# Arthur151/ROMP

Measured on NVIDIA H100. Metric: frames/sec 512x512 ROMP-HRNet32 (whole hot path), higher is better.
Workload: dtype bf16

## Files before the change

romp_b200/_lib.py:

```python
from __future__ import annotations

import ctypes as C
import os
import subprocess
import sys

HERE = os.path.dirname(os.path.abspath(__file__))
ROOT = os.path.dirname(HERE)
LIB_PATH = os.path.join(HERE, "lib", "libb200romp.so")
CSRC = os.path.join(HERE, "csrc")
SOURCES = ["net.cu", "conv_simt.cu", "conv_tc.cu", "conv_stem_tc.cu", "conv1d_tc.cu", "parse.cu", "smpl.cu", "smpl_blend_tc.cu", "project.cu", "bev.cu", "pack.cu", "preproc.cu", "temporal.cu", "resnet_ops.cu"]

F32, BF16, U8 = 0, 1, 2
ENGINE_AUTO, ENGINE_SIMT, ENGINE_TCGEN05, ENGINE_TF32 = 0, 1, 2, 3


class ConvDesc(C.Structure):
    _fields_ = [(n, C.c_int) for n in (
        "in_", "in_c_off", "out", "out_c_off", "res", "res_c_off", "res_broadcast", "cin", "cout",
        "ksize", "stride", "relu", "upsample", "input_norm", "pow_channel", "engine")]


class SumDesc(C.Structure):
    _fields_ = [("out", C.c_int), ("base", C.c_int), ("n_terms", C.c_int), ("term", C.c_int * 4), ("up", C.c_int * 4),
                ("relu", C.c_int), ("term_c_off", C.c_int * 4)]


class BevWeights(C.Structure):
    _fields_ = [(n, C.POINTER(C.c_float)) for n in (
        "center_ref", "cam_ref", "coordmap", "anchors", "embed", "w0", "b0", "w1", "b1", "w2", "b2")]


NVCC_FLAGS = ["-Xcompiler", "-fPIC", "-std=c++17", "-O3", "-lineinfo", "-gencode", "arch=compute_90a,code=sm_90a"]
OBJ_DIR = os.path.join(HERE, "lib", "obj")


def _nvcc():
    return os.environ.get("NVCC", "/usr/local/cuda/bin/nvcc")


def nvcc_command(out_path=LIB_PATH):
    return [_nvcc(), "-shared"] + NVCC_FLAGS + ["-o", out_path] + [os.path.join(CSRC, s) for s in SOURCES]


def _headers_mtime():
    hs = [os.path.join(CSRC, f) for f in os.listdir(CSRC) if f.endswith((".cuh", ".h"))]
    hs.append(os.path.join(ROOT, "include", "b200romp.h"))
    return max(os.path.getmtime(h) for h in hs)


def needs_build():
    if not os.path.exists(LIB_PATH):
        return True
    t = os.path.getmtime(LIB_PATH)
    deps = [os.path.join(CSRC, f) for f in os.listdir(CSRC)] + [os.path.join(ROOT, "include", "b200romp.h")]
    return any(os.path.getmtime(d) > t for d in deps)


def build(force=False, verbose=True):
    if not force and not needs_build():
        return LIB_PATH
    from concurrent.futures import ThreadPoolExecutor
    os.makedirs(OBJ_DIR, exist_ok=True)
    hdr_t = _headers_mtime()
    jobs = []
    for s in SOURCES:
        src, obj = os.path.join(CSRC, s), os.path.join(OBJ_DIR, s.replace(".cu", ".o"))
        if force or not os.path.exists(obj) or os.path.getmtime(obj) < max(os.path.getmtime(src), hdr_t):
            jobs.append([_nvcc(), "-c"] + NVCC_FLAGS + ["-o", obj, src])
    if verbose:
        for j in jobs:
            print("[romp_b200] " + " ".join(j), file=sys.stderr)

    def run(cmd):
        r = subprocess.run(cmd, capture_output=True, text=True)
        if r.returncode != 0:
            raise RuntimeError("nvcc failed: " + " ".join(cmd) + "\n" + r.stdout + r.stderr)
        if verbose and r.stderr.strip():
            print(r.stderr, file=sys.stderr)

    with ThreadPoolExecutor(max_workers=min(len(jobs) or 1, os.cpu_count() or 4)) as ex:
        list(ex.map(run, jobs))
    link = [_nvcc(), "-shared", "-gencode", "arch=compute_90a,code=sm_90a", "-o", LIB_PATH] + [os.path.join(OBJ_DIR, s.replace(".cu", ".o")) for s in SOURCES]
    if verbose:
        print("[romp_b200] " + " ".join(link), file=sys.stderr)
    subprocess.run(link, check=True)
    return LIB_PATH


_lib = None


def _sig(fn, restype, *argtypes):
    fn.restype = restype
# ... 84 lines not shown
```

romp_b200/csrc/conv_tc.cuh:

```cuda
#pragma once
#include <cuda.h>

#include <string>
#include <vector>

#include "common.cuh"

namespace b200romp {

struct S2Maps {
  CUtensorMap m[4];
};

struct TcConvPlan {
  int kind = 0;
  int cin = 0, cout = 0, nt = 0;
  int eb = 2;
  int grid_x = 0, grid_y = 0, stages = 0;
  int smem_bytes = 0;
  void* d_wpack = nullptr;
  alignas(64) unsigned char tmap_in[128];
  alignas(64) unsigned char tmap_s2[4][128];
  unsigned kmask = 0xFFFFFFFFu;
  const void* encoded_in = nullptr;
  int encoded_batch = 0;
  std::string describe() const;
};

bool tc_conv_supported(const ConvParams& p, int ksize, int stride);
int tc_conv_prepare(const ConvParams& p, int ksize, int stride, const float* w_oihw, int sm_count, bool ptrs_final, TcConvPlan* plan,
                    std::vector<void*>* allocs);
int tc_conv_launch(const TcConvPlan& plan, const ConvParams& p, cudaStream_t stream);
bool tc_conv1d_supported(const ConvParams& p);
int tc_conv1d_prepare(const ConvParams& p, const float* w_oi3, int sm_count, TcConvPlan* plan, std::vector<void*>* allocs);
int tc_conv1d_launch(TcConvPlan& plan, const ConvParams& p, cudaStream_t stream);
bool tc_stem_supported(const ConvParams& p, int ksize, int stride);
int tc_stem_prepare(const ConvParams& p, const float* w_oihw, int sm_count, bool out_final, TcConvPlan* plan,
                    std::vector<void*>* allocs);
int tc_stem_launch(const TcConvPlan& plan, const ConvParams& p, cudaStream_t stream);

}
```

romp_b200/csrc/net.cu:

```cuda
#include <stdarg.h>
#include <stdlib.h>
#include <string.h>

#include <algorithm>
#include <map>
#include <mutex>
#include <vector>

#include "common.cuh"
#include "conv_tc.cuh"

namespace b200romp {

static thread_local std::string g_last_error;

void set_error(const char* fmt, ...) {
  char buf[1024];
  va_list ap;
  va_start(ap, fmt);
  vsnprintf(buf, sizeof(buf), fmt, ap);
  va_end(ap);
  g_last_error = buf;
}

struct Tensor {
  int H, W, C, dtype, nchw, external;
  void* ptr = nullptr;
  bool constant = false;
  int first_def = -1, last_use = -1;
  size_t frame_bytes() const { return (size_t)H * W * C * dtype_size(dtype); }
};

struct Op {
  int kind = 0;
  b200romp_sum_desc sum;
  b200romp_conv_desc d;
  std::vector<float> w_host, b_host;
  float* d_w_simt = nullptr;
  float* d_bias = nullptr;
  int coutPad = 0;
  int engine = B200ROMP_ENGINE_SIMT;
  TcConvPlan tc;
  int lane = 0;
  int fold = 0;
};

}

using namespace b200romp;

struct b200romp_net {
  int device = 0;
  int sm_count = 132;
  bool finalized = false;
  int max_batch = 0;
  std::vector<Tensor> tensors;
  std::vector<Op> ops;
  std::vector<void*> device_allocs;
  char* workspace = nullptr;
  size_t workspace_bytes = 0;
  struct GraphKey {
    int batch;
    std::vector<void*> ext;
    bool operator<(const GraphKey& o) const { return batch != o.batch ? batch < o.batch : ext < o.ext; }
  };
  std::map<GraphKey, cudaGraphExec_t> graphs;
  bool use_graph = true;
  static constexpr int kLanes = 4;
  cudaStream_t lane_stream[kLanes] = {nullptr, nullptr, nullptr, nullptr};
  std::vector<cudaEvent_t> op_done;
  cudaEvent_t fork_ev = nullptr;
  bool use_lanes = false;
};

static int fill_params(b200romp_net* net, const Op& op, int batch, ConvParams* out) {
  const b200romp_conv_desc& d = op.d;
  const Tensor& ti = net->tensors[d.in];
  const Tensor& to = net->tensors[d.out];
  ConvParams p;
  memset(&p, 0, sizeof(p));
  p.in = ti.ptr; p.out = to.ptr;
  p.w = op.d_w_simt; p.bias = op.d_bias;
  p.B = batch;
  p.Hin = ti.H; p.Win = ti.W; p.in_C = ti.C; p.in_c_off = d.in_c_off; p.cin = d.cin;
  conv_out_hw(d.ksize, d.stride, ti.H, ti.W, &p.Hout, &p.Wout);
  p.out_C = to.C; p.out_c_off = d.out_c_off; p.cout = d.cout; p.coutPad = op.coutPad;
  p.up = d.upsample;
  if (d.res >= 0) {
    const Tensor& tr = net->tensors[d.res];
    p.res = tr.ptr; p.res_C = tr.C; p.res_c_off = op.d.res_c_off; p.res_broadcast = d.res_broadcast;
    p.res_dtype = tr.dtype;
  }
  p.relu = d.relu; p.pow_channel = d.pow_channel; p.out_nchw = to.nchw;
  p.in_dtype = ti.dtype; p.out_dtype = to.dtype; p.input_norm = d.input_norm;
  if (op.fold) {
    p.Win /= 2; p.Wout /= 2;
    p.in_C *= 2; p.cin *= 2; p.out_C *= 2; p.cout *= 2; p.res_C *= 2;
  }
  if (!p.in || !p.out) {
    set_error("op uses an unbound tensor (in=%d out=%d)", d.in, d.out);
    return B200ROMP_ESTATE;
  }
  *out = p;
  return B200ROMP_OK;
}

static int validate_desc(const std::vector<Tensor>& T, const b200romp_conv_desc& d) {
  const int res_c_off = d.res_c_off;
  auto ok_id = [&](int id) { return id >= 0 && id < (int)T.size(); };
  B2R_REQUIRE(ok_id(d.in) && ok_id(d.out) && (d.res == -1 || ok_id(d.res)), "conv: bad tensor id");
  B2R_REQUIRE((d.ksize == 1 || d.ksize == 3 || d.ksize == 7 || (d.ksize == 13 && d.stride == 1 && d.upsample == 1) ||
               (d.ksize == 42 && d.stride == 2 && d.upsample == 1)) && (d.stride == 1 || d.stride == 2),
              "conv: ksize/stride unsupported");
  B2R_REQUIRE(d.upsample == 1 || d.upsample == 2 || d.upsample == 4 || d.upsample == 8, "conv: upsample must be 1,2,4,8");
  const Tensor& ti = T[d.in];
  const Tensor& to = T[d.out];
  B2R_REQUIRE(!ti.nchw, "conv: NCHW inputs unsupported");
  B2R_REQUIRE(d.cin > 0 && d.in_c_off >= 0 && d.in_c_off + d.cin <= ti.C, "conv: input channel slice out of range");
  B2R_REQUIRE(d.cout > 0 && d.out_c_off >= 0 && d.out_c_off + d.cout <= to.C, "conv: output channel slice out of range");
  int Ho, Wo;
  conv_out_hw(d.ksize, d.stride, ti.H, ti.W, &Ho, &Wo);
  B2R_REQUIRE(Ho * d.upsample == to.H && Wo * d.upsample == to.W, "conv: output tensor is %dx%d, op produces %dx%d",
              to.H, to.W, Ho * d.upsample, Wo * d.upsample);
  B2R_REQUIRE(ti.dtype != B200ROMP_U8 || d.input_norm || d.ksize == 7, "conv: u8 input requires input_norm (or the 7x7 stem)");
  B2R_REQUIRE(to.dtype != B200ROMP_U8, "conv: u8 output unsupported");
  B2R_REQUIRE(!to.nchw || to.dtype == B200ROMP_F32, "conv: NCHW output must be fp32");
  if (d.res >= 0) {
// ... 84 lines not shown
  return (int)net->ops.size() - 1;
}

int b200romp_net_add_sum(b200romp_net* net, const b200romp_sum_desc* desc) {
  B2R_REQUIRE(net && desc && !net->finalized, "add_sum: bad arguments or net already finalized");
  const auto& T = net->tensors;
  const int nT = (int)T.size();
  B2R_REQUIRE(desc->out >= 0 && desc->out < nT && desc->base >= 0 && desc->base < nT, "add_sum: tensor id out of range");
  B2R_REQUIRE(desc->n_terms >= 1 && desc->n_terms <= 4, "add_sum: n_terms must be 1..4");
  const Tensor& to = T[desc->out];
  const Tensor& tb = T[desc->base];
  B2R_REQUIRE(!to.nchw && !tb.nchw && to.dtype != B200ROMP_U8 && tb.dtype != B200ROMP_U8, "add_sum: NHWC bf16/fp32 tensors only");
  B2R_REQUIRE(to.C % 8 == 0 && tb.H == to.H && tb.W == to.W && tb.C == to.C, "add_sum: base/out shape mismatch (C %% 8 == 0)");
  for (int k = 0; k < desc->n_terms; ++k) {
    B2R_REQUIRE(desc->term[k] >= 0 && desc->term[k] < nT, "add_sum: term tensor id out of range");
    const Tensor& tt = T[desc->term[k]];
    const int u = desc->up[k];
    B2R_REQUIRE(u == 1 || u == 2 || u == 4 || u == 8, "add_sum: up must be 1,2,4,8");
    const int co = desc->term_c_off[k];
    B2R_REQUIRE(!tt.nchw && tt.dtype != B200ROMP_U8 && tt.C % 8 == 0 && co >= 0 && co % 8 == 0 && co + to.C <= tt.C &&
                    tt.H * u == to.H && tt.W * u == to.W,
                "add_sum: term %d is %dx%dx%d (slice from channel %d), expected %dx%dx%d", k, tt.H, tt.W, tt.C, co, to.H / u, to.W / u, to.C);
  }
  Op op;
  op.kind = 1;
  op.sum = *desc;
  memset(&op.d, 0, sizeof(op.d));
  op.d.out = desc->out; op.d.in = desc->base; op.d.res = -1;
  net->ops.push_back(std::move(op));
  return (int)net->ops.size() - 1;
}

int b200romp_net_add_maxpool(b200romp_net* net, int in, int out) {
  B2R_REQUIRE(net && !net->finalized, "add_maxpool: net is null or finalized");
  const int nT = (int)net->tensors.size();
  B2R_REQUIRE(in >= 0 && in < nT && out >= 0 && out < nT, "add_maxpool: tensor id out of range");
  const Tensor& ti = net->tensors[in];
  const Tensor& to = net->tensors[out];
  B2R_REQUIRE(!ti.nchw && !to.nchw && ti.dtype == to.dtype && ti.dtype != B200ROMP_U8 && ti.C == to.C, "add_maxpool: NHWC bf16/fp32 tensors of equal C");
  B2R_REQUIRE(to.H == (ti.H + 2 - 3) / 2 + 1 && to.W == (ti.W + 2 - 3) / 2 + 1, "add_maxpool: output must be %dx%d", (ti.H - 1) / 2 + 1, (ti.W - 1) / 2 + 1);
  Op op;
  op.kind = 2;
  memset(&op.d, 0, sizeof(op.d));
  memset(&op.sum, 0, sizeof(op.sum));
  op.d.in = in; op.d.out = out; op.d.res = -1;
  net->ops.push_back(std::move(op));
  return (int)net->ops.size() - 1;
}

static int fill_sum_params(b200romp_net* net, const Op& op, int batch, SumParams* out) {
  SumParams p;
  memset(&p, 0, sizeof(p));
  const Tensor& to = net->tensors[op.sum.out];
  const Tensor& tb = net->tensors[op.sum.base];
  B2R_REQUIRE(to.ptr && tb.ptr, "sum op: unbound tensor");
  p.base = tb.ptr; p.base_dt = tb.dtype; p.out = to.ptr; p.out_dt = to.dtype;
  p.n_terms = op.sum.n_terms;
  for (int k = 0; k < p.n_terms; ++k) {
    const Tensor& tt = net->tensors[op.sum.term[k]];
    B2R_REQUIRE(tt.ptr, "sum op: unbound term tensor");
    p.term[k] = tt.ptr; p.term_dt[k] = tt.dtype; p.up[k] = op.sum.up[k];
    p.term_C[k] = tt.C; p.term_c_off[k] = op.sum.term_c_off[k];
  }
  p.B = batch; p.H = to.H; p.W = to.W; p.C = to.C; p.relu = op.sum.relu;
  *out = p;
  return B200ROMP_OK;
}

static int enqueue_op(b200romp_net* net, Op& op, int batch, cudaStream_t stream) {
  if (op.kind == 1) {
    SumParams sp;
    int rc = fill_sum_params(net, op, batch, &sp);
    return rc ? rc : launch_fuse_sum(sp, stream);
  }
  if (op.kind == 2) {
    const Tensor& ti = net->tensors[op.d.in];
    const Tensor& to = net->tensors[op.d.out];
    B2R_REQUIRE(ti.ptr && to.ptr, "maxpool op: unbound tensor");
    return launch_maxpool3x3s2(ti.ptr, to.ptr, ti.dtype, batch, ti.H, ti.W, ti.C, stream);
  }
  ConvParams p;
  int rc = fill_params(net, op, batch, &p);
  if (rc) return rc;
  if (op.d.ksize == 7) return launch_conv_generic(p, 7, op.d.stride, stream);
  if (op.d.ksize == 42) return launch_deconv4x4s2(p, stream);
  if (op.engine == B200ROMP_ENGINE_TCGEN05) return op.tc.kind == 13 ? tc_conv1d_launch(op.tc, p, stream) : tc_conv_launch(op.tc, p, stream);
  return launch_conv_simt(p, op.d.ksize, op.d.stride, stream);
}

static int upload_simt_weights(b200romp_net* net, Op& op) {
  const b200romp_conv_desc& d = op.d;
  const int taps = conv_taps(d.ksize);
  op.coutPad = (d.cout + 63) / 64 * 64;
  std::vector<float> packed((size_t)taps * d.cin * op.coutPad, 0.f);
  for (int co = 0; co < d.cout; ++co)
    for (int ci = 0; ci < d.cin; ++ci)
      for (int t = 0; t < taps; ++t)
        packed[((size_t)t * d.cin + ci) * op.coutPad + co] =
            d.ksize == 42 ? op.w_host[((size_t)ci * d.cout + co) * taps + t] : op.w_host[((size_t)co * d.cin + ci) * taps + t];
  std::vector<float> bias(op.coutPad, 0.f);
  std::copy(op.b_host.begin(), op.b_host.end(), bias.begin());
  B2R_CUDA_OK(cudaMalloc(&op.d_w_simt, packed.size() * sizeof(float)));
  net->device_allocs.push_back(op.d_w_simt);
  B2R_CUDA_OK(cudaMemcpy(op.d_w_simt, packed.data(), packed.size() * sizeof(float), cudaMemcpyHostToDevice));
  B2R_CUDA_OK(cudaMalloc(&op.d_bias, bias.size() * sizeof(float)));
  net->device_allocs.push_back(op.d_bias);
  B2R_CUDA_OK(cudaMemcpy(op.d_bias, bias.data(), bias.size() * sizeof(float), cudaMemcpyHostToDevice));
  return B200ROMP_OK;
}

static bool fold_eligible(const b200romp_net* net, const Op& op) {
  static const bool off = [] { const char* e = getenv("B200ROMP_TC_NO_FOLD"); return e && e[0] == '1'; }();
  const b200romp_conv_desc& d = op.d;
  const Tensor& ti = net->tensors[d.in];
  const Tensor& to = net->tensors[d.out];
  if (off || d.ksize != 3 || d.stride != 1 || d.upsample != 1 || d.cin != 32 || d.cout != 32) return false;
  if (ti.C != 32 || to.C != 32 || d.in_c_off || d.out_c_off || ti.external || to.external) return false;
  if (ti.dtype != B200ROMP_BF16 || to.dtype != B200ROMP_BF16 || to.nchw || d.pow_channel >= 0 || d.input_norm) return false;
  if (ti.W % 16 != 0 || ti.H % 16 != 0) return false;
  if (d.res >= 0) {
    const Tensor& tr = net->tensors[d.res];
    if (tr.C != 32 || d.res_c_off || d.res_broadcast || tr.dtype != B200ROMP_BF16 || tr.external) return false;
  }
  return true;
}

static void fold_pixel_pairs(const std::vector<float>& w, const std::vector<float>& b, std::vector<float>* w2, std::vector<float>* b2,
                             unsigned* kmask) {
  w2->assign((size_t)64 * 64 * 9, 0.f);
  for (int dx = 0; dx < 2; ++dx)
    for (int co = 0; co < 32; ++co)
      for (int h = 0; h < 2; ++h)
        for (int ci = 0; ci < 32; ++ci)
          for (int ky = 0; ky < 3; ++ky)
            for (int s = -1; s <= 1; ++s) {
              const int kx = 2 * s + h - dx + 1;
              if (kx < 0 || kx > 2) continue;
              (*w2)[(((size_t)(dx * 32 + co) * 64 + h * 32 + ci) * 3 + ky) * 3 + (s + 1)] = w[(((size_t)co * 32 + ci) * 3 + ky) * 3 + kx];
            }
  b2->assign(64, 0.f);
  for (int i = 0; i < 64; ++i) (*b2)[i] = (i % 32) < (int)b.size() ? b[i % 32] : 0.f;
  unsigned m = 0;
  for (int t = 0; t < 9; ++t) {
    const int s = t % 3 - 1;
    if (s != -1) m |= 1u << (t * 2 + 0);
    if (s != +1) m |= 1u << (t * 2 + 1);
  }
  *kmask = m;
}

int b200romp_net_finalize(b200romp_net* net, int max_batch) {
  B2R_REQUIRE(net && !net->finalized && max_batch > 0, "finalize: bad arguments");
  B2R_CUDA_OK(cudaSetDevice(net->device));
  const int nT = (int)net->tensors.size(), nO = (int)net->ops.size();
  for (int i = 0; i < nO; ++i) {
    const b200romp_conv_desc& d = net->ops[i].d;
    Tensor& to = net->tensors[d.out];
    if (to.first_def < 0) to.first_def = i;
    to.last_use = std::max(to.last_use, i);
    net->tensors[d.in].last_use = std::max(net->tensors[d.in].last_use, i);
    if (d.res >= 0) net->tensors[d.res].last_use = std::max(net->tensors[d.res].last_use, i);
    if (net->ops[i].kind == 1)
      for (int k = 0; k < net->ops[i].sum.n_terms; ++k) {
        Tensor& tt = net->tensors[net->ops[i].sum.term[k]];
        B2R_REQUIRE(tt.external || tt.constant || (tt.first_def >= 0 && tt.first_def < i), "op %d sums tensor %d before it is written", i, net->ops[i].sum.term[k]);
        tt.last_use = std::max(tt.last_use, i);
      }
  }
  for (int i = 0; i < nO; ++i) {
    const b200romp_conv_desc& d = net->ops[i].d;
    const Tensor& ti = net->tensors[d.in];
    B2R_REQUIRE(ti.external || ti.constant || (ti.first_def >= 0 && ti.first_def < i), "op %d reads tensor %d before it is written", i, d.in);
    if (d.res >= 0) {
      const Tensor& tr = net->tensors[d.res];
      B2R_REQUIRE(tr.external || tr.constant || (tr.first_def >= 0 && tr.first_def < i), "op %d adds tensor %d before it is written", i, d.res);
    }
  }
  struct Buf { size_t bytes; size_t offset; };
  std::vector<Buf> bufs;
  std::multimap<size_t, int> free_bufs;
  std::vector<int> tensor_buf(nT, -1);
  std::vector<std::vector<int>> dies_at(nO);
  for (int t = 0; t < nT; ++t) {
    const Tensor& tt = net->tensors[t];
    if (!tt.external && !tt.constant && tt.first_def >= 0) dies_at[tt.last_use].push_back(t);
  }
  size_t total = 0;
  for (int i = 0; i < nO; ++i) {
    const int t = net->ops[i].d.out;
    const Tensor& tt = net->tensors[t];
    if (!tt.external && !tt.constant && tt.first_def == i) {
      const size_t bytes = (tt.frame_bytes() * max_batch + 1023) / 1024 * 1024;
      auto it = free_bufs.find(bytes);
      if (it != free_bufs.end()) {
        tensor_buf[t] = it->second;
        free_bufs.erase(it);
      } else {
        bufs.push_back({bytes, total});
        total += bytes;
        tensor_buf[t] = (int)bufs.size() - 1;
      }
    }
    for (int dead : dies_at[i]) free_bufs.insert({bufs[tensor_buf[dead]].bytes, tensor_buf[dead]});
  }
  if (total > 0) {
    B2R_CUDA_OK(cudaMalloc(&net->workspace, total));
    B2R_CUDA_OK(cudaMemset(net->workspace, 0, total));
  }
  net->workspace_bytes = total;
  for (int t = 0; t < nT; ++t)
    if (tensor_buf[t] >= 0) net->tensors[t].ptr = net->workspace + bufs[tensor_buf[t]].offset;
  net->max_batch = max_batch;
  for (int i = 0; i < nO; ++i) {
    Op& op = net->ops[i];
    if (op.kind == 1 || op.kind == 2) continue;
    int rc = upload_simt_weights(net, op);
    if (rc) return rc;
    op.engine = B200ROMP_ENGINE_SIMT;
    const Tensor& ti = net->tensors[op.d.in];
    const Tensor& to = net->tensors[op.d.out];
    const bool stem_like = ti.dtype == B200ROMP_U8 && op.d.cin == 3 && op.d.ksize == 3 && op.d.stride == 2;
    if (op.d.ksize == 7 || op.d.ksize == 42) { op.w_host.clear(); op.w_host.shrink_to_fit(); continue; }
    const bool want_tf32 = op.d.engine == B200ROMP_ENGINE_TF32 && ti.dtype == B200ROMP_F32;
    const bool want_tc = op.d.engine == B200ROMP_ENGINE_TCGEN05 || want_tf32 ||
                         (op.d.engine == B200ROMP_ENGINE_AUTO && (ti.dtype == B200ROMP_BF16 || stem_like));
    if (want_tc) {
      ConvParams p;
      bool ext_out_unbound = false, ext_in_unbound = false;
      if (to.external && to.ptr == nullptr) {
        net->tensors[op.d.out].ptr = reinterpret_cast<void*>(16);
        ext_out_unbound = true;
      }
      const bool conv1d = op.d.ksize == 13;
      if ((stem_like || conv1d) && ti.external && ti.ptr == nullptr) {
        net->tensors[op.d.in].ptr = reinterpret_cast<void*>(16);
        ext_in_unbound = true;
      }
      const bool params_ok = (!ti.external || stem_like || conv1d) && fill_params(net, op, max_batch, &p) == B200ROMP_OK;
      if (ext_out_unbound) net->tensors[op.d.out].ptr = nullptr;
      if (ext_in_unbound) net->tensors[op.d.in].ptr = nullptr;
      const bool ptrs_final = !to.external && (op.d.res < 0 || !net->tensors[op.d.res].external);
      if (params_ok && stem_like && ptrs_final && tc_stem_supported(p, op.d.ksize, op.d.stride)) {
        rc = tc_stem_prepare(p, op.w_host.data(), net->sm_count, ptrs_final, &op.tc, &net->device_allocs);
        if (rc == B200ROMP_OK) op.engine = B200ROMP_ENGINE_TCGEN05;
        else if (op.d.engine == B200ROMP_ENGINE_TCGEN05) return rc;
      } else if (params_ok && conv1d && ti.dtype == B200ROMP_BF16 && tc_conv1d_supported(p)) {
        rc = tc_conv1d_prepare(p, op.w_host.data(), net->sm_count, &op.tc, &net->device_allocs);
        if (rc == B200ROMP_OK) op.engine = B200ROMP_ENGINE_TCGEN05;
        else if (op.d.engine == B200ROMP_ENGINE_TCGEN05) return rc;
      } else if (params_ok && !stem_like && !conv1d && (ti.dtype != B200ROMP_F32 || want_tf32 || op.d.engine == B200ROMP_ENGINE_TCGEN05) &&
                 tc_conv_supported(p, op.d.ksize, op.d.stride)) {
        rc = -1;
        if (fold_eligible(net, op)) {
          std::vector<float> w2, b2;
          unsigned kmask = 0;
          fold_pixel_pairs(op.w_host, op.b_host, &w2, &b2, &kmask);
          ConvParams pf;
          op.fold = 1;
          TcConvPlan plan;
          if (fill_params(net, op, max_batch, &pf) == B200ROMP_OK && tc_conv_supported(pf, 3, 1) &&
              tc_conv_prepare(pf, 3, 1, w2.data(), net->sm_count, ptrs_final, &plan, &net->device_allocs) == B200ROMP_OK && plan.kind == 30 && plan.nt == 64) {
            plan.kmask = kmask;
            op.tc = plan;
            B2R_CUDA_OK(cudaMemcpy(op.d_bias, b2.data(), 64 * sizeof(float), cudaMemcpyHostToDevice));
            rc = B200ROMP_OK;
          } else {
            op.fold = 0;
          }
        }
        if (rc != B200ROMP_OK)
          rc = tc_conv_prepare(p, op.d.ksize, op.d.stride, op.w_host.data(), net->sm_count, ptrs_final, &op.tc, &net->device_allocs);
        if (rc == B200ROMP_OK) op.engine = B200ROMP_ENGINE_TCGEN05;
        else if (op.d.engine == B200ROMP_ENGINE_TCGEN05) return rc;
      } else if (op.d.engine == B200ROMP_ENGINE_TCGEN05) {
        set_error("op %d: tensor-core engine forced but shape unsupported", i);
        return B200ROMP_EINVAL;
      }
    }
    op.w_host.clear(); op.w_host.shrink_to_fit();
  }
  net->finalized = true;
  return B200ROMP_OK;
}

int b200romp_net_bind(b200romp_net* net, int tensor, void* device_ptr) {
  B2R_REQUIRE(net && tensor >= 0 && tensor < (int)net->tensors.size(), "bind: bad tensor id");
  B2R_REQUIRE(net->tensors[tensor].external, "bind: tensor %d is not external", tensor);
  net->tensors[tensor].ptr = device_ptr;
  return B200ROMP_OK;
}

static int enqueue_all_lanes(b200romp_net* net, int batch, cudaStream_t stream) {
  constexpr int L = b200romp_net::kLanes;
  const size_t n = net->ops.size();
  if (net->op_done.size() != n) {
    for (cudaEvent_t e : net->op_done) cudaEventDestroy(e);
    net->op_done.assign(n, nullptr);
    for (auto& e : net->op_done) B2R_CUDA_OK(cudaEventCreateWithFlags(&e, cudaEventDisableTiming));
// ... 63 lines not shown
  B2R_REQUIRE(batch > 0 && batch <= net->max_batch, "run: batch %d outside 1..%d", batch, net->max_batch);
  cudaStream_t stream = (cudaStream_t)stream_;
  B2R_CUDA_OK(cudaSetDevice(net->device));
  if (!net->use_graph || stream == nullptr) return enqueue_all(net, batch, stream);
  b200romp_net::GraphKey key;
  key.batch = batch;
  for (const Tensor& t : net->tensors)
    if (t.external) key.ext.push_back(t.ptr);
  auto it = net->graphs.find(key);
  if (it == net->graphs.end()) {
    cudaGraph_t graph = nullptr;
    cudaError_t e = cudaStreamBeginCapture(stream, cudaStreamCaptureModeThreadLocal);
    if (e != cudaSuccess) {
      cudaGetLastError();
      return enqueue_all(net, batch, stream);
    }
    bool lanes = false;
    if (net->use_lanes)
      for (const Op& op : net->ops) lanes = lanes || op.lane != 0;
    int rc = lanes ? enqueue_all_lanes(net, batch, stream) : enqueue_all(net, batch, stream);
    e = cudaStreamEndCapture(stream, &graph);
    if (rc) {
      if (graph) cudaGraphDestroy(graph);
      return rc;
    }
    B2R_CUDA_OK(e);
    cudaGraphExec_t exec = nullptr;
    B2R_CUDA_OK(cudaGraphInstantiate(&exec, graph, 0));
    cudaGraphDestroy(graph);
    if (net->graphs.size() >= 16) {
      B2R_CUDA_OK(cudaStreamSynchronize(stream));
      for (auto& kv : net->graphs) cudaGraphExecDestroy(kv.second);
      net->graphs.clear();
    }
    it = net->graphs.insert({key, exec}).first;
  }
  B2R_CUDA_OK(cudaGraphLaunch(it->second, stream));
  return B200ROMP_OK;
}

int b200romp_net_profile(b200romp_net* net, int batch, int iters, float* us_per_op, b200romp_stream stream_) {
  B2R_REQUIRE(net && net->finalized && us_per_op && iters > 0, "profile: bad arguments");
  B2R_REQUIRE(batch > 0 && batch <= net->max_batch, "profile: batch %d outside 1..%d", batch, net->max_batch);
  cudaStream_t stream = (cudaStream_t)stream_;
  B2R_CUDA_OK(cudaSetDevice(net->device));
  const size_t n = net->ops.size();
  std::vector<cudaEvent_t> ev(n + 1);
  for (auto& e : ev) B2R_CUDA_OK(cudaEventCreate(&e));
  std::vector<double> acc(n, 0.0);
  int rc = B200ROMP_OK;
  for (int it = 0; it < iters + 1 && rc == B200ROMP_OK; ++it) {
    cudaEventRecord(ev[0], stream);
    for (size_t i = 0; i < n && rc == B200ROMP_OK; ++i) {
      rc = enqueue_op(net, net->ops[i], batch, stream);
      cudaEventRecord(ev[i + 1], stream);
    }
    if (rc) break;
    if (cudaStreamSynchronize(stream) != cudaSuccess) { set_error("profile: %s", cudaGetErrorString(cudaGetLastError())); rc = B200ROMP_ECUDA; break; }
    if (it == 0) continue;
    for (size_t i = 0; i < n; ++i) {
      float ms = 0.f;
      cudaEventElapsedTime(&ms, ev[i], ev[i + 1]);
      acc[i] += ms * 1000.0;
    }
  }
  for (auto& e : ev) cudaEventDestroy(e);
  if (rc) return rc;
  for (size_t i = 0; i < n; ++i) us_per_op[i] = (float)(acc[i] / iters);
  return B200ROMP_OK;
}

int b200romp_net_read_tensor(b200romp_net* net, int tensor, int batch, void* dst, b200romp_stream stream) {
  B2R_REQUIRE(net && net->finalized && tensor >= 0 && tensor < (int)net->tensors.size(), "read_tensor: bad arguments");
  const Tensor& t = net->tensors[tensor];
  B2R_REQUIRE(t.ptr != nullptr, "read_tensor: tensor %d has no storage", tensor);
  const size_t bytes = t.frame_bytes() * (t.constant ? 1 : batch);
  B2R_CUDA_OK(cudaMemcpyAsync(dst, t.ptr, bytes, cudaMemcpyDeviceToDevice, (cudaStream_t)stream));
  return B200ROMP_OK;
}

int b200romp_net_describe(b200romp_net* net, char* buf, int len) {
  if (!net || !buf || len <= 0) return B200ROMP_EINVAL;
  std::string s;
  char line[256];
  for (size_t i = 0; i < net->ops.size(); ++i) {
    const Op& op = net->ops[i];
    const b200romp_conv_desc& d = op.d;
    const Tensor& ti = net->tensors[d.in];
    const Tensor& to = net->tensors[d.out];
    if (op.kind == 2) {
      snprintf(line, sizeof(line), "op%03zu maxpool 3x3 s2 in t%d[%dx%dx%d] out t%d[%dx%dx%d]\n", i, d.in, ti.H, ti.W, ti.C, d.out, to.H, to.W, to.C);
      s += line;
      continue;
    }
    if (op.kind == 1) {
      int n = snprintf(line, sizeof(line), "op%03zu sum     out t%d[%dx%dx%d] = relu%d( t%d", i, op.sum.out, to.H, to.W, to.C, op.sum.relu, op.sum.base);
      for (int k = 0; k < op.sum.n_terms; ++k) n += snprintf(line + n, sizeof(line) - n, " + up%d(t%d)", op.sum.up[k], op.sum.term[k]);
      snprintf(line + n, sizeof(line) - n, " )\n");
      s += line;
      continue;
    }
    snprintf(line, sizeof(line), "op%03zu %s k%d s%d %4d->%-4d in t%d[%dx%dx%d]+%d out t%d[%dx%dx%d]+%d res t%d up%d relu%d%s\n", i,
             op.engine == B200ROMP_ENGINE_TCGEN05 ? "wgmma  " : "simt   ", d.ksize, d.stride, d.cin, d.cout, d.in, ti.H,
             ti.W, ti.C, d.in_c_off, d.out, to.H, to.W, to.C, d.out_c_off, d.res, d.upsample, d.relu,
             op.engine == B200ROMP_ENGINE_TCGEN05 ? op.tc.describe().c_str() : "");
    s += line;
  }
  snprintf(line, sizeof(line), "workspace %.1f MiB for max_batch %d\n", net->workspace_bytes / 1048576.0, net->max_batch);
  s += line;
  const int n = (int)std::min<size_t>(s.size(), (size_t)len - 1);
  memcpy(buf, s.data(), n);
  buf[n] = 0;
  return n;
}

int b200romp_net_set_lane(b200romp_net* net, int op, int lane) {
  B2R_REQUIRE(net && !net->finalized && op >= 0 && op < (int)net->ops.size(), "set_lane: bad op id or net already finalized");
  B2R_REQUIRE(lane >= 0 && lane < b200romp_net::kLanes, "set_lane: lane must be 0..%d", b200romp_net::kLanes - 1);
  net->ops[op].lane = lane;
  return B200ROMP_OK;
}

int b200romp_net_num_launches(b200romp_net* net) { return net ? (int)net->ops.size() : 0; }
long long b200romp_net_workspace_bytes(b200romp_net* net) { return net ? (long long)net->workspace_bytes : 0; }

int b200romp_conv2d(const b200romp_conv_desc* d, const float* weight_host, const float* bias_host, const void* in,
                    int in_dtype, int in_H, int in_W, int in_C, void* out, int out_dtype, int out_C, int out_nchw,
                    const void* res, int res_dtype, int batch, b200romp_stream stream) {
  B2R_REQUIRE(d && weight_host && in && out && batch > 0, "conv2d: bad arguments");
  int dev = 0;
  B2R_CUDA_OK(cudaGetDevice(&dev));
  b200romp_net* net = b200romp_net_create(dev);
  if (!net) return B200ROMP_ECUDA;
  int Ho, Wo;
  conv_out_hw(d->ksize, d->stride, in_H, in_W, &Ho, &Wo);
  Ho *= d->upsample; Wo *= d->upsample;
  b200romp_conv_desc dd = *d;
  dd.in = b200romp_net_add_tensor(net, in_H, in_W, in_C, in_dtype, 0, 1);
  dd.out = b200romp_net_add_tensor(net, Ho, Wo, out_C, out_dtype, out_nchw, 1);
  dd.res = -1;
  if (res) dd.res = b200romp_net_add_tensor(net, Ho, Wo, out_C, res_dtype, 0, 1);
  int rc = (dd.in < 0 || dd.out < 0) ? B200ROMP_EINVAL : B200ROMP_OK;
  if (!rc) {
    net->tensors[dd.in].ptr = const_cast<void*>(in);
    net->tensors[dd.out].ptr = out;
    if (res) net->tensors[dd.res].ptr = const_cast<void*>(res);
    net->tensors[dd.in].external = net->tensors[dd.out].external = 0;
    if (res) net->tensors[dd.res].external = 0;
    net->tensors[dd.in].constant = true;
    net->tensors[dd.out].constant = true;
    if (res) net->tensors[dd.res].constant = true;
    dd.res_c_off = d->out_c_off;
    rc = b200romp_net_add_conv(net, &dd, weight_host, bias_host);
    rc = rc < 0 ? rc : B200ROMP_OK;
  }
  if (!rc) rc = b200romp_net_finalize(net, batch);
  if (!rc) {
    net->use_graph = false;
    rc = b200romp_net_run(net, batch, stream);
  }
  if (!rc) {
    cudaError_t e = cudaStreamSynchronize((cudaStream_t)stream);
    if (e != cudaSuccess) {
      set_error("conv2d: %s", cudaGetErrorString(e));
      rc = B200ROMP_ECUDA;
    }
  }
  b200romp_net_destroy(net);
  return rc;
}

}
```

Baseline: 3058.

## Fuse HRNet basic-block conv pairs into one warp-specialized wgmma kernel

Adds a fused kernel that runs both 3x3 convs of an HRNet basic block (64 or pixel-pair-folded 32 channels) in one persistent launch. The intermediate activation stays in shared memory, computed over a halo tile, and the residual is read from the already-loaded input tile. A graph pass at finalize merges eligible consecutive conv ops into a single block op. This removes the global-memory round trip for the mid tensor and one launch per block, at the cost of recomputing halo pixels, a single-stage TMA pipeline and only one CTA per SM because of the large shared-memory footprint.

```diff
diff --git a/romp_b200/_lib.py b/romp_b200/_lib.py
--- a/romp_b200/_lib.py
+++ b/romp_b200/_lib.py
@@ -9,7 +9,7 @@
 ROOT = os.path.dirname(HERE)
 LIB_PATH = os.path.join(HERE, "lib", "libb200romp.so")
 CSRC = os.path.join(HERE, "csrc")
-SOURCES = ["net.cu", "conv_simt.cu", "conv_tc.cu", "conv_stem_tc.cu", "conv1d_tc.cu", "parse.cu", "smpl.cu", "smpl_blend_tc.cu", "project.cu", "bev.cu", "pack.cu", "preproc.cu", "temporal.cu", "resnet_ops.cu"]
+SOURCES = ["net.cu", "conv_simt.cu", "conv_tc.cu", "conv_block_tc.cu", "conv_stem_tc.cu", "conv1d_tc.cu", "parse.cu", "smpl.cu", "smpl_blend_tc.cu", "project.cu", "bev.cu", "pack.cu", "preproc.cu", "temporal.cu", "resnet_ops.cu"]
 
 F32, BF16, U8 = 0, 1, 2
 ENGINE_AUTO, ENGINE_SIMT, ENGINE_TCGEN05, ENGINE_TF32 = 0, 1, 2, 3
diff --git a/romp_b200/csrc/conv_block_tc.cu b/romp_b200/csrc/conv_block_tc.cu
--- /dev/null
+++ b/romp_b200/csrc/conv_block_tc.cu
@@ -0,0 +1,263 @@
+#include "conv_tc.cuh"
+#include "tc_device.cuh"
+
+namespace b200romp {
+
+namespace {
+
+constexpr int kBlkThreads = 384;
+constexpr int kRowB = 128;
+constexpr int kHaloW = 12, kHaloH = 20;
+constexpr int kTapBytes = 64 * kRowB;
+constexpr int kWBytes = 9 * kTapBytes;
+constexpr int kStagePayload = kHaloH * kHaloW * kRowB;
+constexpr int kStageBytes = (282 * kRowB + 1023) / 1024 * 1024;
+constexpr int kMidBytes = 256 * kRowB;
+constexpr int kSmemBytes = 2 * kWBytes + kStageBytes + kMidBytes + 1024  + 1024 ;
+static_assert(kSmemBytes <= 227 * 1024, "fused block does not fit shared memory");
+
+template <bool FOLD>
+__device__ __forceinline__ constexpr bool blk_skip(int tap, int k) {
+  return FOLD && ((tap % 3 == 0 && k < 2) || (tap % 3 == 2 && k >= 2));
+}
+
+__device__ __forceinline__ void consumers_bar_sync() { asm volatile("bar.sync 1, 256;" ::: "memory"); }
+
+__device__ __forceinline__ uint32_t ld_shared_b32(uint32_t addr) {
+  uint32_t v;
+  asm volatile("ld.shared.b32 %0, [%1];" : "=r"(v) : "r"(addr));
+  return v;
+}
+__device__ __forceinline__ void st_shared_b32(uint32_t addr, uint32_t v) {
+  asm volatile("st.shared.b32 [%0], %1;" ::"r"(addr), "r"(v) : "memory");
+}
+template <typename T>
+__device__ __forceinline__ T opaque(T v) {
+  uint64_t u = (uint64_t)v;
+  asm volatile("mov.b64 %0, %0;" : "+l"(u));
+  return (T)u;
+}
+__device__ __forceinline__ uint32_t pack_bf16x2(float a, float b) {
+  const __nv_bfloat162 v = __floats2bfloat162_rn(a, b);
+  return *reinterpret_cast<const uint32_t*>(&v);
+}
+
+}
+
+template <bool FOLD>
+__global__ void __launch_bounds__(kBlkThreads, 1)
+conv_block_tc_kernel(const __grid_constant__ CUtensorMap tmap, const ConvParams p, const uint8_t* __restrict__ w1pack,
+                     const uint8_t* __restrict__ w2pack, const float* __restrict__ bias1, int tiles_x, int tiles_y, int num_tiles) {
+  extern __shared__ uint8_t smem_raw[];
+  uint8_t* smem = reinterpret_cast<uint8_t*>((reinterpret_cast<uintptr_t>(smem_raw) + 1023) & ~(uintptr_t)1023);
+  uint8_t* sW1 = smem;
+  uint8_t* sW2 = smem + kWBytes;
+  uint8_t* sA = smem + 2 * kWBytes;
+  uint8_t* sMid = sA + kStageBytes;
+  uint64_t* full = reinterpret_cast<uint64_t*>(sMid + kMidBytes);
+  uint64_t* empty = full + 1;
+  uint64_t* w_full = full + 2;
+
+  const int warp = threadIdx.x >> 5;
+  if (threadIdx.x == 0) {
+    mbar_init(full, 1);
+    mbar_init(empty, 256);
+    mbar_init(w_full, 1);
+    fence_barrier_init();
+  }
+  __syncthreads();
+  pdl_trigger();
+  const int per_frame = tiles_x * tiles_y;
+
+  if (warp == 0) {
+    if (elect_one()) {
+      mbar_arrive_expect_tx(w_full, 2 * kWBytes);
+      for (int t = 0; t < 9; ++t) {
+        bulk_copy_g2s(sW1 + t * kTapBytes, w1pack + (size_t)t * kTapBytes, kTapBytes, w_full);
+        bulk_copy_g2s(sW2 + t * kTapBytes, w2pack + (size_t)t * kTapBytes, kTapBytes, w_full);
+      }
+      pdl_wait();
+      const uint64_t pol = l2_policy_stream();
+      uint32_t phase = 0;
+      for (int tile = blockIdx.x; tile < num_tiles; tile += gridDim.x, phase ^= 1) {
+        const int n = tile / per_frame, rem = tile % per_frame;
+        const int y0 = (rem / tiles_x) * 16, x0 = (rem % tiles_x) * 8;
+        mbar_wait(empty, phase ^ 1);
+        mbar_arrive_expect_tx(full, kStagePayload);
+        tma_load_4d(sA, &tmap, full, 0, x0 - 2, y0 - 2, n, pol);
+      }
+    }
+  } else if (warp >= 4) {
+    const int g = (warp >> 2) - 1, t = threadIdx.x & 127, w = t >> 5, l = t & 31;
+    pdl_wait();
+    mbar_wait(w_full, 0);
+    const int cl = 2 * (l & 3);
+    uint32_t phase = 0;
+    for (int tile = blockIdx.x; tile < num_tiles; tile += gridDim.x, phase ^= 1) {
+      const uint32_t w1_base = opaque(smem_u32(sW1)), w2_base = opaque(smem_u32(sW2)), a_base = opaque(smem_u32(sA)),
+                     mid_base = opaque(smem_u32(sMid));
+      const float* b1p = opaque(bias1);
+      const float* b2p = opaque(p.bias);
+      const int n = tile / per_frame, rem = tile % per_frame;
+      const int y0 = (rem / tiles_x) * 16, x0 = (rem % tiles_x) * 8;
+      mbar_wait(full, phase);
+
+      float acc[2][32];
+#pragma unroll
+      for (int h = 0; h < 2; ++h)
+#pragma unroll
+        for (int j = 0; j < 32; ++j) acc[h][j] = 0.f;
+      uint32_t scale_d = 0;
+      wgmma_fence();
+#pragma unroll
+      for (int tap = 0; tap < 9; ++tap) {
+        const uint32_t a_tap = a_base + (uint32_t)((128 * g + (tap / 3) * kHaloW + tap % 3) * kRowB);
+        const uint32_t b_tap = w1_base + (uint32_t)(tap * kTapBytes);
+#pragma unroll
+        for (int k = 0; k < 4; ++k) {
+          if (blk_skip<FOLD>(tap, k)) continue;
+          const uint64_t bdesc = make_smem_desc(b_tap + k * 32, 8 * kRowB, kSw128);
+          wgmma_n64(acc[0], make_smem_desc(a_tap + k * 32, 8 * kRowB, kSw128), bdesc, scale_d, false);
+          wgmma_n64(acc[1], make_smem_desc(a_tap + 64 * kRowB + k * 32, 8 * kRowB, kSw128), bdesc, scale_d, false);
+          scale_d = 1;
+        }
+      }
+      wgmma_commit();
+      uint32_t rv[2][8];
+#pragma unroll
+      for (int e = 0; e < 2; ++e) {
+        const int hr = (8 * g + 2 * w + e + 2) * kHaloW + (l >> 2) + 2;
+#pragma unroll
+        for (int j = 0; j < 8; ++j) rv[e][j] = ld_shared_b32(a_base + hr * kRowB + ((j ^ (hr & 7)) << 4) + 2 * cl);
+      }
+      wgmma_wait<0>();
+      mbar_arrive(empty);
+
+      consumers_bar_sync();
+#pragma unroll
+      for (int h = 0; h < 2; ++h) {
+#pragma unroll
+        for (int e = 0; e < 2; ++e) {
+          const int m = 64 * (2 * g + h) + 16 * w + (l >> 2) + 8 * e;
+          const int my = m / kHaloW, mx = m % kHaloW;
+          const bool inside = my < 18 && mx < 10 && (unsigned)(y0 - 1 + my) < (unsigned)p.Hout && (unsigned)(x0 - 1 + mx) < (unsigned)p.Wout;
+          const uint32_t row = mid_base + m * kRowB;
+#pragma unroll
+          for (int j = 0; j < 8; ++j) {
+            const int c = 8 * j + cl;
+            float a = fmaxf(acc[h][4 * j + 2 * e] + __ldg(b1p + c), 0.f);
+            float b = fmaxf(acc[h][4 * j + 2 * e + 1] + __ldg(b1p + c + 1), 0.f);
+            if (!inside) a = b = 0.f;
+            st_shared_b32(row + ((j ^ (m & 7)) << 4) + 2 * cl, pack_bf16x2(a, b));
+          }
+        }
+      }
+      fence_proxy_async();
+      consumers_bar_sync();
+
+      float acc2[32];
+#pragma unroll
+      for (int j = 0; j < 32; ++j) acc2[j] = 0.f;
+      scale_d = 0;
+      wgmma_fence();
+#pragma unroll
+      for (int tap = 0; tap < 9; ++tap) {
+        const uint32_t a_tap = mid_base + (uint32_t)(((8 * g + tap / 3) * kHaloW + tap % 3) * kRowB);
+        const uint32_t b_tap = w2_base + (uint32_t)(tap * kTapBytes);
+#pragma unroll
+        for (int k = 0; k < 4; ++k) {
+          if (blk_skip<FOLD>(tap, k)) continue;
+          wgmma_n64(acc2, make_smem_desc(a_tap + k * 32, kHaloW * kRowB, kSw128), make_smem_desc(b_tap + k * 32, 8 * kRowB, kSw128),
+                    scale_d, false);
+          scale_d = 1;
+        }
+      }
+      wgmma_commit();
+      wgmma_wait<0>();
+
+      __nv_bfloat16* out = reinterpret_cast<__nv_bfloat16*>(p.out);
+#pragma unroll
+      for (int e = 0; e < 2; ++e) {
+        const size_t pix = ((size_t)n * p.Hout + y0 + 8 * g + 2 * w + e) * p.Wout + x0 + (l >> 2);
+        __nv_bfloat162* o = reinterpret_cast<__nv_bfloat162*>(out + pix * p.out_C + p.out_c_off + cl);
+#pragma unroll
+        for (int j = 0; j < 8; ++j) {
+          const int c = 8 * j + cl;
+          float a = acc2[4 * j + 2 * e] + __ldg(b2p + c), b = acc2[4 * j + 2 * e + 1] + __ldg(b2p + c + 1);
+          const float2 r = res_pair(rv[e][j]);
+          a += r.x; b += r.y;
+          o[4 * j] = __floats2bfloat162_rn(fmaxf(a, 0.f), fmaxf(b, 0.f));
+        }
+      }
+    }
+  }
+}
+
+bool tc_block_supported(const ConvParams& p) {
+  if (p.in_dtype != B200ROMP_BF16 || p.out_dtype != B200ROMP_BF16 || p.res_dtype != B200ROMP_BF16) return false;
+  if (p.cin != 64 || p.cout != 64 || p.up != 1 || p.out_nchw || p.pow_channel >= 0 || p.input_norm || !p.relu) return false;
+  if (p.Hin != p.Hout || p.Win != p.Wout || p.Hout % 16 != 0 || p.Wout % 8 != 0) return false;
+  if (p.in_C % 8 != 0 || p.in_c_off % 8 != 0 || p.out_C % 8 != 0 || p.out_c_off % 8 != 0) return false;
+  if (p.res != p.in || p.res_C != p.in_C || p.res_c_off != p.in_c_off || p.res_broadcast) return false;
+  return (reinterpret_cast<uintptr_t>(p.in) & 15) == 0;
+}
+
+int tc_block_prepare(const ConvParams& p, const float* w1_oihw, const float* b1, const float* w2_oihw, bool fold, int sm_count,
+                     TcConvPlan* plan, std::vector<void*>* allocs) {
+  if (!tc_block_supported(p)) {
+    set_error("conv_block_tc: unsupported block shape");
+    return B200ROMP_EINVAL;
+  }
+  PFN_encodeTiled encode = tc_get_encode();
+  if (!encode) {
+    set_error("conv_block_tc: cuTensorMapEncodeTiled is unavailable");
+    return B200ROMP_ECUDA;
+  }
+  plan->kind = 60;
+  plan->eb = 2;
+  plan->cin = plan->cout = plan->nt = 64;
+  plan->grid_x = sm_count;
+  plan->grid_y = 1;
+  plan->stages = 1;
+  plan->smem_bytes = kSmemBytes;
+  plan->fold = fold ? 1 : 0;
+  int rc = tc_pack_weights(w1_oihw, 64, 64, 9, 64, &plan->d_wpack, allocs, kRowB, 2);
+  if (rc) return rc;
+  rc = tc_pack_weights(w2_oihw, 64, 64, 9, 64, &plan->d_wpack2, allocs, kRowB, 2);
+  if (rc) return rc;
+  void* db1 = nullptr;
+  B2R_CUDA_OK(cudaMalloc(&db1, 64 * sizeof(float)));
+  allocs->push_back(db1);
+  B2R_CUDA_OK(cudaMemcpy(db1, b1, 64 * sizeof(float), cudaMemcpyHostToDevice));
+  plan->d_bias1 = static_cast<const float*>(db1);
+  CUtensorMap tm;
+  const cuuint64_t gdim[4] = {64, (cuuint64_t)p.Win, (cuuint64_t)p.Hin, (cuuint64_t)p.B};
+  const cuuint64_t gstr[3] = {(cuuint64_t)p.in_C * 2, (cuuint64_t)p.Win * p.in_C * 2, (cuuint64_t)p.Hin * p.Win * p.in_C * 2};
+  const cuuint32_t box[4] = {64, kHaloW, kHaloH, 1};
+  const cuuint32_t estr[4] = {1, 1, 1, 1};
+  void* base = const_cast<uint8_t*>(static_cast<const uint8_t*>(p.in) + (size_t)p.in_c_off * 2);
+  CUresult cr = encode(&tm, CU_TENSOR_MAP_DATA_TYPE_BFLOAT16, 4, base, gdim, gstr, box, estr, CU_TENSOR_MAP_INTERLEAVE_NONE,
+                       CU_TENSOR_MAP_SWIZZLE_128B, CU_TENSOR_MAP_L2_PROMOTION_L2_128B, CU_TENSOR_MAP_FLOAT_OOB_FILL_NONE);
+  if (cr != CUDA_SUCCESS) {
+    set_error("conv_block_tc: cuTensorMapEncodeTiled failed with %d", (int)cr);
+    return B200ROMP_ECUDA;
+  }
+  memcpy(plan->tmap_in, &tm, sizeof(tm));
+  B2R_CUDA_OK(cudaFuncSetAttribute(conv_block_tc_kernel<false>, cudaFuncAttributeMaxDynamicSharedMemorySize, kSmemBytes));
+  B2R_CUDA_OK(cudaFuncSetAttribute(conv_block_tc_kernel<true>, cudaFuncAttributeMaxDynamicSharedMemorySize, kSmemBytes));
+  return B200ROMP_OK;
+}
+
+int tc_block_launch(const TcConvPlan& plan, const ConvParams& p, cudaStream_t stream) {
+  CUtensorMap tm;
+  memcpy(&tm, plan.tmap_in, sizeof(tm));
+  const int tiles_x = p.Wout / 8, tiles_y = p.Hout / 16;
+  const int num_tiles = tiles_x * tiles_y * p.B;
+  const dim3 grid(std::min(plan.grid_x, num_tiles));
+  auto kern = plan.fold ? conv_block_tc_kernel<true> : conv_block_tc_kernel<false>;
+  B2R_CUDA_OK(tc_launch(kern, grid, kBlkThreads, plan.smem_bytes, stream, tm, p, reinterpret_cast<const uint8_t*>(plan.d_wpack),
+                        reinterpret_cast<const uint8_t*>(plan.d_wpack2), plan.d_bias1, tiles_x, tiles_y, num_tiles));
+  return B200ROMP_OK;
+}
+
+}
diff --git a/romp_b200/csrc/conv_tc.cuh b/romp_b200/csrc/conv_tc.cuh
--- a/romp_b200/csrc/conv_tc.cuh
+++ b/romp_b200/csrc/conv_tc.cuh
@@ -24,6 +24,9 @@
   unsigned kmask = 0xFFFFFFFFu;
   const void* encoded_in = nullptr;
   int encoded_batch = 0;
+  void* d_wpack2 = nullptr;
+  const float* d_bias1 = nullptr;
+  int fold = 0;
   std::string describe() const;
 };
 
@@ -38,5 +41,9 @@
 int tc_stem_prepare(const ConvParams& p, const float* w_oihw, int sm_count, bool out_final, TcConvPlan* plan,
                     std::vector<void*>* allocs);
 int tc_stem_launch(const TcConvPlan& plan, const ConvParams& p, cudaStream_t stream);
+bool tc_block_supported(const ConvParams& p);
+int tc_block_prepare(const ConvParams& p, const float* w1_oihw, const float* b1, const float* w2_oihw, bool fold, int sm_count,
+                     TcConvPlan* plan, std::vector<void*>* allocs);
+int tc_block_launch(const TcConvPlan& plan, const ConvParams& p, cudaStream_t stream);
 
 }
diff --git a/romp_b200/csrc/net.cu b/romp_b200/csrc/net.cu
--- a/romp_b200/csrc/net.cu
+++ b/romp_b200/csrc/net.cu
@@ -43,6 +43,9 @@
   TcConvPlan tc;
   int lane = 0;
   int fold = 0;
+  int block = 0;
+  int mid = -1;
+  std::vector<float> w2_host, b2_host;
 };
 
 }
@@ -293,6 +296,7 @@
   ConvParams p;
   int rc = fill_params(net, op, batch, &p);
   if (rc) return rc;
+  if (op.block) return tc_block_launch(op.tc, p, stream);
   if (op.d.ksize == 7) return launch_conv_generic(p, 7, op.d.stride, stream);
   if (op.d.ksize == 42) return launch_deconv4x4s2(p, stream);
   if (op.engine == B200ROMP_ENGINE_TCGEN05) return op.tc.kind == 13 ? tc_conv1d_launch(op.tc, p, stream) : tc_conv_launch(op.tc, p, stream);
@@ -360,9 +364,99 @@
   *kmask = m;
 }
 
+static bool is_bf16_block_conv(const b200romp_net* net, const Op& op) {
+  const b200romp_conv_desc& d = op.d;
+  const Tensor& ti = net->tensors[d.in];
+  const Tensor& to = net->tensors[d.out];
+  return op.kind == 0 && d.ksize == 3 && d.stride == 1 && d.upsample == 1 && d.relu && !d.input_norm && d.pow_channel < 0 &&
+         (d.engine == B200ROMP_ENGINE_AUTO || d.engine == B200ROMP_ENGINE_TCGEN05) && ti.dtype == B200ROMP_BF16 &&
+         to.dtype == B200ROMP_BF16 && !to.nchw && d.cin == d.cout && (d.cin == 64 || d.cin == 32);
+}
+
+static void fuse_basic_blocks(b200romp_net* net) {
+  const int nT = (int)net->tensors.size();
+  std::vector<int> reads(nT, 0), writes(nT, 0);
+  for (const Op& op : net->ops) {
+    ++reads[op.d.in];
+    ++writes[op.d.out];
+    if (op.kind == 1)
+      for (int k = 0; k < op.sum.n_terms; ++k) ++reads[op.sum.term[k]];
+    else if (op.d.res >= 0) ++reads[op.d.res];
+  }
+  std::vector<Op> fused;
+  fused.reserve(net->ops.size());
+  for (size_t i = 0; i < net->ops.size(); ++i) {
+    Op& a = net->ops[i];
+    if (i + 1 < net->ops.size()) {
+      Op& b = net->ops[i + 1];
+      const int x = a.d.in, t = a.d.out;
+      const Tensor& tx = net->tensors[x];
+      const Tensor& tt = net->tensors[t];
+      const int C = a.d.cin;
+      bool ok = is_bf16_block_conv(net, a) && is_bf16_block_conv(net, b) && a.d.res < 0 && b.d.cin == C && a.lane == b.lane &&
+                b.d.in == t && b.d.in_c_off == 0 && a.d.out_c_off == 0 && tt.C == C && !tt.external && !tt.constant &&
+                reads[t] == 1 && writes[t] == 1 && b.d.res == x && b.d.res_c_off == a.d.in_c_off && !b.d.res_broadcast &&
+                !tx.external && tx.H % 16 == 0;
+      bool fold = false;
+      if (ok && C == 32) {
+        fold = fold_eligible(net, a) && fold_eligible(net, b);
+        ok = fold;
+      }
+      if (ok && C == 64) {
+        const Tensor& ty = net->tensors[b.d.out];
+        ok = !ty.external && tx.W % 8 == 0 && tx.C % 8 == 0 && a.d.in_c_off % 8 == 0 && ty.C % 8 == 0 && b.d.out_c_off % 8 == 0;
+      }
+      if (ok) {
+        Op f;
+        f.d = a.d;
+        f.d.out = b.d.out;
+        f.d.out_c_off = b.d.out_c_off;
+        f.d.res = x;
+        f.d.res_c_off = b.d.res_c_off;
+        f.block = 1;
+        f.fold = fold ? 1 : 0;
+        f.mid = t;
+        f.lane = a.lane;
+        f.w_host = std::move(a.w_host);
+        f.b_host = std::move(a.b_host);
+        f.w2_host = std::move(b.w_host);
+        f.b2_host = std::move(b.b_host);
+        fused.push_back(std::move(f));
+        ++i;
+        continue;
+      }
+    }
+    fused.push_back(std::move(a));
+  }
+  net->ops = std::move(fused);
+}
+
+static int prepare_block(b200romp_net* net, Op& op, int max_batch) {
+  std::vector<float> w1 = op.w_host, b1 = op.b_host, w2 = op.w2_host, b2 = op.b2_host;
+  if (op.fold) {
+    unsigned kmask = 0;
+    fold_pixel_pairs(op.w_host, op.b_host, &w1, &b1, &kmask);
+    fold_pixel_pairs(op.w2_host, op.b2_host, &w2, &b2, &kmask);
+  }
+  op.coutPad = 64;
+  B2R_CUDA_OK(cudaMalloc(&op.d_bias, 64 * sizeof(float)));
+  net->device_allocs.push_back(op.d_bias);
+  B2R_CUDA_OK(cudaMemcpy(op.d_bias, b2.data(), 64 * sizeof(float), cudaMemcpyHostToDevice));
+  ConvParams p;
+  int rc = fill_params(net, op, max_batch, &p);
+  if (rc) return rc;
+  rc = tc_block_prepare(p, w1.data(), b1.data(), w2.data(), op.fold != 0, net->sm_count, &op.tc, &net->device_allocs);
+  if (rc) return rc;
+  op.engine = B200ROMP_ENGINE_TCGEN05;
+  op.w_host.clear(); op.w_host.shrink_to_fit();
+  op.w2_host.clear(); op.w2_host.shrink_to_fit();
+  return B200ROMP_OK;
+}
+
 int b200romp_net_finalize(b200romp_net* net, int max_batch) {
   B2R_REQUIRE(net && !net->finalized && max_batch > 0, "finalize: bad arguments");
   B2R_CUDA_OK(cudaSetDevice(net->device));
+  fuse_basic_blocks(net);
   const int nT = (int)net->tensors.size(), nO = (int)net->ops.size();
   for (int i = 0; i < nO; ++i) {
     const b200romp_conv_desc& d = net->ops[i].d;
@@ -425,6 +519,11 @@
   for (int i = 0; i < nO; ++i) {
     Op& op = net->ops[i];
     if (op.kind == 1 || op.kind == 2) continue;
+    if (op.block) {
+      int rc = prepare_block(net, op, max_batch);
+      if (rc) return rc;
+      continue;
+    }
     int rc = upload_simt_weights(net, op);
     if (rc) return rc;
     op.engine = B200ROMP_ENGINE_SIMT;
@@ -654,7 +753,7 @@
 int b200romp_net_describe(b200romp_net* net, char* buf, int len) {
   if (!net || !buf || len <= 0) return B200ROMP_EINVAL;
   std::string s;
-  char line[256];
+  char line[384];
   for (size_t i = 0; i < net->ops.size(); ++i) {
     const Op& op = net->ops[i];
     const b200romp_conv_desc& d = op.d;
@@ -669,6 +768,16 @@
       int n = snprintf(line, sizeof(line), "op%03zu sum     out t%d[%dx%dx%d] = relu%d( t%d", i, op.sum.out, to.H, to.W, to.C, op.sum.relu, op.sum.base);
       for (int k = 0; k < op.sum.n_terms; ++k) n += snprintf(line + n, sizeof(line) - n, " + up%d(t%d)", op.sum.up[k], op.sum.term[k]);
       snprintf(line + n, sizeof(line) - n, " )\n");
+      s += line;
+      continue;
+    }
+    if (op.block) {
+      const Tensor& tm = net->tensors[op.mid];
+      snprintf(line, sizeof(line),
+               "op%03zu wgmma   block k3 s1 %d->%d->%d in t%d[%dx%dx%d]+%d mid t%d[%dx%dx%d] out t%d[%dx%dx%d]+%d res t%d+%d up1 relu1 "
+               "bias1 bias2 [tc-block grid %d smem %d%s]\n",
+               i, d.cin, d.cin, d.cout, d.in, ti.H, ti.W, ti.C, d.in_c_off, op.mid, tm.H, tm.W, tm.C, d.out, to.H, to.W, to.C,
+               d.out_c_off, d.res, d.res_c_off, op.tc.grid_x, op.tc.smem_bytes, op.fold ? " conv1 pixel-pairs conv2 pixel-pairs" : "");
       s += line;
       continue;
     }
```

Result: faster. 3201 (median of 6 runs) (+4.7%).
